# Okrio/tinyrecurrentunet

Measured on AMD Instinct MI355X. Metric: 16 kHz frames/sec (train step), higher is better.
Workload: dtype f32; 1 GPU; config/tiny.json TRU-Net (C_in=4 incl. PCEN), 64 x 4 s 16 kHz pairs per GPU, n_fft 512 hop 128, full fp32 train step; mfma=fp32 forward, bf16x3 backward, fp32_mfma=bf16x3-bwd, frames_per_gpu=32064, global_batch=64, parallelism=dp1

## Files before the change

tinyrecurrentunet_amd/csrc/elementwise.hip:

```cpp
#include <stdlib.h>
#include "common.hpp"

namespace {

__global__ void to_frames_last_kernel(const float* __restrict__ x, float* __restrict__ y, int N, int R, int NP) {
    __shared__ float t[32][33];
    const int n0 = blockIdx.x * 32, r0 = blockIdx.y * 32;
    const int tx = threadIdx.x, ty = threadIdx.y;
    for (int i = ty; i < 32; i += 8) {
        int n = n0 + i, r = r0 + tx;
        t[i][tx] = (n < N && r < R) ? x[(size_t)n * R + r] : 0.f;
    }
    __syncthreads();
    for (int i = ty; i < 32; i += 8) {
        int r = r0 + i, n = n0 + tx;
        if (r < R && n < NP) y[(size_t)r * NP + n] = t[tx][i];
    }
}

__global__ void from_frames_last_kernel(const float* __restrict__ y, float* __restrict__ x, int N, int R, int NP) {
    __shared__ float t[32][33];
    const int n0 = blockIdx.x * 32, r0 = blockIdx.y * 32;
    const int tx = threadIdx.x, ty = threadIdx.y;
    for (int i = ty; i < 32; i += 8) {
        int r = r0 + i, n = n0 + tx;
        t[i][tx] = (r < R && n < NP) ? y[(size_t)r * NP + n] : 0.f;
    }
    __syncthreads();
    for (int i = ty; i < 32; i += 8) {
        int n = n0 + i, r = r0 + tx;
        if (n < N && r < R) x[(size_t)n * R + r] = t[tx][i];
    }
}

__global__ void from_frames_last_affine_kernel(const float* __restrict__ y, float* __restrict__ x, int N, int R, int NP,
                                               int L, const float* __restrict__ scale, const float* __restrict__ shift,
                                               float lo) {
    __shared__ float t[32][33];
    const int n0 = blockIdx.x * 32, r0 = blockIdx.y * 32;
    const int tx = threadIdx.x, ty = threadIdx.y;
    for (int i = ty; i < 32; i += 8) {
        int r = r0 + i, n = n0 + tx;
        float v = 0.f;
        if (r < R && n < NP) {
            const int c = r / L;
            v = fmaxf(fmaf(y[(size_t)r * NP + n], scale[c], shift[c]), lo);
        }
        t[i][tx] = v;
    }
    __syncthreads();
    for (int i = ty; i < 32; i += 8) {
        int n = n0 + i, r = r0 + tx;
        if (n < N && r < R) x[(size_t)n * R + r] = t[tx][i];
    }
}

template <int CIN, int K>
__global__ __launch_bounds__(256) void conv_first_kernel(const float* __restrict__ x, const float* __restrict__ w,
                                                         const float* __restrict__ b, float* __restrict__ y, int Cout,
                                                         int S, int Lin, int Lout, int NP) {
    const int f4 = threadIdx.x;
    const int lo = blockIdx.y * 8 + threadIdx.y;
    const size_t n = (size_t)blockIdx.x * 128 + 4 * f4;
    if (lo >= Lout) return;
    f32x4 xv[CIN][K];
#pragma unroll
    for (int ci = 0; ci < CIN; ++ci)
#pragma unroll
        for (int k = 0; k < K; ++k) {
            int li = lo * S + k - S / 2;
            f32x4 z = {0.f, 0.f, 0.f, 0.f};
            xv[ci][k] = (li >= 0 && li < Lin) ? *(const f32x4*)(x + ((size_t)ci * Lin + li) * NP + n) : z;
        }
    for (int co = 0; co < Cout; ++co) {
        const float bb = b[co];
        f32x4 acc = {bb, bb, bb, bb};
#pragma unroll
        for (int ci = 0; ci < CIN; ++ci)
#pragma unroll
            for (int k = 0; k < K; ++k) {
                const float wv = w[(co * CIN + ci) * K + k];
#pragma unroll
                for (int e = 0; e < 4; ++e) acc[e] = fmaf(wv, xv[ci][k][e], acc[e]);
            }
#pragma unroll
        for (int e = 0; e < 4; ++e) acc[e] = fmaxf(acc[e], 0.f);
#ifdef TRUNET_THIN_NT
        __builtin_nontemporal_store(acc, (f32x4*)(y + ((size_t)co * Lout + lo) * NP + n));
#else
        *(f32x4*)(y + ((size_t)co * Lout + lo) * NP + n) = acc;
#endif
    }
}

constexpr int DW_PARTS = 16;

template <int K>
__global__ __launch_bounds__(256) void dwconv_fwd_kernel(const float* __restrict__ zin, const float* __restrict__ s_in,
                                                         const float* __restrict__ t_in, const float* __restrict__ w,
                                                         const float* __restrict__ b, float* __restrict__ zout,
                                                         float* __restrict__ partials, int C, int S, int Lin, int Lout,
                                                         int NP, int N) {
    __shared__ double red[256];
    const int c = blockIdx.y;
    const int f4 = threadIdx.x & 31, ly = threadIdx.x >> 5;
    const float sc = s_in[c], sh = t_in[c], bb = b[c];
    float wk[K];
#pragma unroll
    for (int k = 0; k < K; ++k) wk[k] = w[c * K + k];
    const int ntn = NP / 128;
    const int items = Lout * ntn;
    float s1 = 0.f, s2 = 0.f;
    for (int it = blockIdx.x * 8 + ly; it < items; it += gridDim.x * 8) {
        const int nt = it / Lout, lo = it - nt * Lout;
// ... 17 lines not shown
    double r2 = block_sum_f64((double)s2, red);
    if (threadIdx.x == 0) {
        partials[((size_t)blockIdx.x * C + c) * 2 + 0] = (float)r1;
        partials[((size_t)blockIdx.x * C + c) * 2 + 1] = (float)r2;
    }
}

template <int K>
__global__ __launch_bounds__(256) void dwconv_bwd_kernel(
    const float* __restrict__ dy, const float* __restrict__ z, const float* __restrict__ ca,
    const float* __restrict__ cb, const float* __restrict__ cc, const float* __restrict__ zin,
    const float* __restrict__ s_in, const float* __restrict__ t_in, const float* __restrict__ mean_in,
    const float* __restrict__ w, float* __restrict__ dy_in, float* __restrict__ partials_in,
    float* __restrict__ w_partials, float* __restrict__ b_partials, int C, int S, int Lin, int Lout, int NP, int N) {
    __shared__ double red[256];
    const int c = blockIdx.y;
    const int f4 = threadIdx.x & 31, ly = threadIdx.x >> 5;
    const float a0 = ca[c], a1 = cb[c], a2 = cc[c];
    const float sc = s_in[c], sh = t_in[c], mu = mean_in[c];
    float wk[K], dwk[K];
#pragma unroll
    for (int k = 0; k < K; ++k) { wk[k] = w[c * K + k]; dwk[k] = 0.f; }
    float db = 0.f, s1 = 0.f, s2 = 0.f;
    const int ntn = NP / 128;
    const int items = Lin * ntn;
    for (int it = blockIdx.x * 8 + ly; it < items; it += gridDim.x * 8) {
        const int nt = it / Lin, li = it - nt * Lin;
        const int n = nt * 128 + 4 * f4;
        const f32x4 zi = *(const f32x4*)(zin + ((size_t)c * Lin + li) * NP + n);
        f32x4 act, g = {0.f, 0.f, 0.f, 0.f};
#pragma unroll
        for (int e = 0; e < 4; ++e) act[e] = fmaxf(fmaf(zi[e], sc, sh), 0.f);
#pragma unroll
        for (int k = 0; k < K; ++k) {
            const int num = li + K / 2 - k;
            const int lo = num / S;
            if (num >= 0 && lo * S == num && lo < Lout) {
                const size_t off = ((size_t)c * Lout + lo) * NP + n;
                const f32x4 dv = *(const f32x4*)(dy + off);
                const f32x4 zv = *(const f32x4*)(z + off);
#pragma unroll
                for (int e = 0; e < 4; ++e) {
                    float dz = (n + e < N) ? fmaf(a0, dv[e], fmaf(a1, zv[e], a2)) : 0.f;
                    g[e] = fmaf(wk[k], dz, g[e]);
                    dwk[k] = fmaf(dz, act[e], dwk[k]);
                    if (k == K / 2) db += dz;
                }
            }
        }
        f32x4 o;
#pragma unroll
        for (int e = 0; e < 4; ++e) {
            o[e] = (act[e] > 0.f) ? g[e] : 0.f;
            s1 += o[e];
            s2 = fmaf(o[e], zi[e] - mu, s2);
        }
        *(f32x4*)(dy_in + ((size_t)c * Lin + li) * NP + n) = o;
    }
    double r;
    r = block_sum_f64((double)s1, red);
    if (threadIdx.x == 0) partials_in[((size_t)blockIdx.x * C + c) * 2 + 0] = (float)r;
    r = block_sum_f64((double)s2, red);
    if (threadIdx.x == 0) partials_in[((size_t)blockIdx.x * C + c) * 2 + 1] = (float)r;
    r = block_sum_f64((double)db, red);
    if (threadIdx.x == 0) b_partials[(size_t)blockIdx.x * C + c] = (float)r;
#pragma unroll
    for (int k = 0; k < K; ++k) {
        r = block_sum_f64((double)dwk[k], red);
        if (threadIdx.x == 0) w_partials[((size_t)blockIdx.x * C + c) * K + k] = (float)r;
    }
}

constexpr int DW2_FB = 32;
constexpr int DW2_CH = 4;
constexpr int DW2_PARTS = DW2_FB * DW2_CH;

#ifndef TRUNET_DW_TEMPORAL
#define DW2_LD(p) __builtin_nontemporal_load((const f32x4*)(p))
#define DW2_ST(p, v) __builtin_nontemporal_store((v), (f32x4*)(p))
#else
#define DW2_LD(p) (*(const f32x4*)(p))
#define DW2_ST(p, v) (*(f32x4*)(p) = (v))
#endif
template <int K, int S>
__global__ __launch_bounds__(256) void dw2_fwd_kernel(const float* __restrict__ zin, const float* __restrict__ s_in,
                                                      const float* __restrict__ t_in, const float* __restrict__ w,
                                                      const float* __restrict__ b, float* __restrict__ zout,
                                                      float* __restrict__ partials, int C, int Lin, int Lout, int NP, int N) {
    __shared__ double red[256];
    const int c = blockIdx.y;
    const float sc = s_in[c], sh = t_in[c], bb = b[c];
    float wk[K];
#pragma unroll
    for (int k = 0; k < K; ++k) wk[k] = w[c * K + k];
    const int lo0 = (int)(((long long)blockIdx.z * Lout) / DW2_CH), lo1 = (int)(((long long)(blockIdx.z + 1) * Lout) / DW2_CH);
    double s1 = 0.0, s2 = 0.0;
    for (int qd = blockIdx.x * 256 + threadIdx.x; qd < NP / 4; qd += DW2_FB * 256) {
        const int n = 4 * qd;
        const float* src = zin + (size_t)c * Lin * NP + n;
        float* dst = zout + (size_t)c * Lout * NP + n;
        auto load_act = [&](int li) {
            f32x4 a = {0.f, 0.f, 0.f, 0.f};
            if (li >= 0 && li < Lin) {
                const f32x4 v = DW2_LD(src + (size_t)li * NP);
#pragma unroll
                for (int e = 0; e < 4; ++e) a[e] = fmaxf(fmaf(v[e], sc, sh), 0.f);
            }
            return a;
        };
        f32x4 win[K];
#pragma unroll
        for (int k = 0; k < K - S; ++k) win[k + S] = load_act(lo0 * S + k - K / 2);
        for (int lo = lo0; lo < lo1; ++lo) {
#pragma unroll
            for (int k = 0; k < K - S; ++k) win[k] = win[k + S];
#pragma unroll
            for (int k = K - S; k < K; ++k) win[k] = load_act(lo * S + k - K / 2);
            f32x4 acc = {bb, bb, bb, bb};
#pragma unroll
            for (int k = 0; k < K; ++k)
#pragma unroll
                for (int e = 0; e < 4; ++e) acc[e] = fmaf(wk[k], win[k][e], acc[e]);
            DW2_ST(dst + (size_t)lo * NP, acc);
            float r1 = 0.f, r2 = 0.f;
#pragma unroll
            for (int e = 0; e < 4; ++e)
                if (n + e < N) { r1 += acc[e]; r2 = fmaf(acc[e], acc[e], r2); }
            s1 += (double)r1;
            s2 += (double)r2;
        }
    }
    const int part = blockIdx.z * DW2_FB + blockIdx.x;
    const double r1 = block_sum_f64(s1, red);
    const double r2 = block_sum_f64(s2, red);
    if (threadIdx.x == 0) {
        partials[((size_t)part * C + c) * 2 + 0] = (float)r1;
        partials[((size_t)part * C + c) * 2 + 1] = (float)r2;
    }
}

template <int K, int S>
__global__ __launch_bounds__(256) void dw2_bwd_kernel(
    const float* __restrict__ dy, const float* __restrict__ z, const float* __restrict__ ca,
    const float* __restrict__ cb, const float* __restrict__ cc, const float* __restrict__ zin,
    const float* __restrict__ s_in, const float* __restrict__ t_in, const float* __restrict__ mean_in,
    const float* __restrict__ w, float* __restrict__ dy_in, float* __restrict__ partials_in,
    float* __restrict__ w_partials, float* __restrict__ b_partials, int C, int Lin, int Lout, int NP, int N) {
    constexpr int LOMIN = -1, LOMAX = 1, W = 3;
    static_assert((K == 3 && S == 1) || (K == 5 && S == 2) || (K == 3 && S == 2), "window derived for these shapes");
    __shared__ double red[256];
    const int c = blockIdx.y;
    const float a0 = ca[c], a1 = cb[c], a2 = cc[c];
    const float sc = s_in[c], sh = t_in[c], mu = mean_in[c];
    float wk[K];
    double dwk[K];
#pragma unroll
    for (int k = 0; k < K; ++k) { wk[k] = w[c * K + k]; dwk[k] = 0.0; }
    double db = 0.0, s1 = 0.0, s2 = 0.0;
    const int G = (Lin + S - 1) / S;
    const int m0 = (int)(((long long)blockIdx.z * G) / DW2_CH), m1 = (int)(((long long)(blockIdx.z + 1) * G) / DW2_CH);
    for (int qd = blockIdx.x * 256 + threadIdx.x; qd < NP / 4; qd += DW2_FB * 256) {
        const int n = 4 * qd;
        const float* pdy = dy + (size_t)c * Lout * NP + n;
        const float* pz = z + (size_t)c * Lout * NP + n;
        const float* pin = zin + (size_t)c * Lin * NP + n;
        float* pout = dy_in + (size_t)c * Lin * NP + n;
        auto load_dz = [&](int lo) {
            f32x4 d = {0.f, 0.f, 0.f, 0.f};
            if (lo >= 0 && lo < Lout) {
                const f32x4 dv = DW2_LD(pdy + (size_t)lo * NP);
                const f32x4 zv = DW2_LD(pz + (size_t)lo * NP);
#pragma unroll
                for (int e = 0; e < 4; ++e) d[e] = (n + e < N) ? fmaf(a0, dv[e], fmaf(a1, zv[e], a2)) : 0.f;
            }
            return d;
        };
        f32x4 dzw[W];
#pragma unroll
        for (int i = 1; i < W; ++i) dzw[i] = load_dz(m0 + LOMIN + i - 1);
        for (int m = m0; m < m1; ++m) {
#pragma unroll
            for (int i = 0; i < W - 1; ++i) dzw[i] = dzw[i + 1];
            dzw[W - 1] = load_dz(m + LOMAX);
#pragma unroll
            for (int e = 0; e < S; ++e) {
                const int li = m * S + e;
                if (li >= Lin) continue;
                const f32x4 zi = DW2_LD(pin + (size_t)li * NP);
                f32x4 act, g = {0.f, 0.f, 0.f, 0.f};
#pragma unroll
                for (int j = 0; j < 4; ++j) act[j] = fmaxf(fmaf(zi[j], sc, sh), 0.f);
#pragma unroll
                for (int k = 0; k < K; ++k) {
                    constexpr int half = K / 2;
                    const int num = e + half - k;
                    if (((num % S) + S) % S != 0) continue;
                    const int lo_rel = (num >= 0) ? num / S : -((-num) / S);
                    const int wi = lo_rel - LOMIN;
                    float rw = 0.f, rb = 0.f;
#pragma unroll
                    for (int j = 0; j < 4; ++j) {
                        const float dzv = dzw[wi][j];
                        g[j] = fmaf(wk[k], dzv, g[j]);
                        rw = fmaf(dzv, act[j], rw);
                        rb += dzv;
                    }
                    dwk[k] += (double)rw;
                    if (k == half) db += (double)rb;
                }
                f32x4 o;
                float r1 = 0.f, r2 = 0.f;
#pragma unroll
                for (int j = 0; j < 4; ++j) {
                    o[j] = (act[j] > 0.f) ? g[j] : 0.f;
                    r1 += o[j];
                    r2 = fmaf(o[j], zi[j] - mu, r2);
                }
                s1 += (double)r1;
                s2 += (double)r2;
                DW2_ST(pout + (size_t)li * NP, o);
            }
        }
    }
    const int part = blockIdx.z * DW2_FB + blockIdx.x;
    double r;
    r = block_sum_f64(s1, red);
    if (threadIdx.x == 0) partials_in[((size_t)part * C + c) * 2 + 0] = (float)r;
    r = block_sum_f64(s2, red);
    if (threadIdx.x == 0) partials_in[((size_t)part * C + c) * 2 + 1] = (float)r;
    r = block_sum_f64(db, red);
    if (threadIdx.x == 0) b_partials[(size_t)part * C + c] = (float)r;
#pragma unroll
    for (int k = 0; k < K; ++k) {
        r = block_sum_f64(dwk[k], red);
        if (threadIdx.x == 0) w_partials[((size_t)part * C + c) * K + k] = (float)r;
    }
}

template <int K, int S>
__global__ __launch_bounds__(256) void dw2_bwd_rz_kernel(
    const float* __restrict__ dy, const float* __restrict__ bias, const float* __restrict__ ca,
    const float* __restrict__ cb, const float* __restrict__ cc, const float* __restrict__ zin,
    const float* __restrict__ s_in, const float* __restrict__ t_in, const float* __restrict__ mean_in,
    const float* __restrict__ w, float* __restrict__ dy_in, float* __restrict__ partials_in,
    float* __restrict__ w_partials, float* __restrict__ b_partials, int C, int Lin, int Lout, int NP, int N) {
    constexpr int LOMIN = -1, W = 3;
    constexpr int AW = S + K / 2 + 1, ZO = S - K / 2;
    static_assert((K == 3 && S == 1) || (K == 5 && S == 2) || (K == 3 && S == 2), "window derived for these shapes");
    __shared__ double red[256];
    const int c = blockIdx.y;
    const float a0 = ca[c], a1 = cb[c], a2 = cc[c];
    const float sc = s_in[c], sh = t_in[c], mu = mean_in[c], bb = bias[c];
    const bool sc0 = fabsf(sc) < 1e-30f || fabsf(sh) > 65536.f * fabsf(sc);
    const float isc = sc0 ? 0.f : 1.f / sc, zoff = fmaf(sh, isc, mu);
    float wk[K];
    double dwk[K];
#pragma unroll
    for (int k = 0; k < K; ++k) { wk[k] = w[c * K + k]; dwk[k] = 0.0; }
    double db = 0.0, s1 = 0.0, s2 = 0.0;
    const int G = (Lin + S - 1) / S;
    const int m0 = (int)(((long long)blockIdx.z * G) / DW2_CH), m1 = (int)(((long long)(blockIdx.z + 1) * G) / DW2_CH);
    for (int qd = blockIdx.x * 256 + threadIdx.x; qd < NP / 4; qd += DW2_FB * 256) {
        const int n = 4 * qd;
        const float* pdy = dy + (size_t)c * Lout * NP + n;
        const float* pin = zin + (size_t)c * Lin * NP + n;
        float* pout = dy_in + (size_t)c * Lin * NP + n;
        f32x4 aw[AW];
        auto load_row = [&](int li, f32x4& act) {
            const bool ok = li >= 0 && li < Lin;
            const f32x4 raw = DW2_LD(pin + (size_t)min(max(li, 0), Lin - 1) * NP);
#pragma unroll
            for (int j = 0; j < 4; ++j) act[j] = ok ? fmaxf(fmaf(raw[j], sc, sh), 0.f) : 0.f;
        };
        f32x4 dzw[W];
#pragma unroll
        for (int i = 0; i < W; ++i) dzw[i] = f32x4{0.f, 0.f, 0.f, 0.f};
        const int ms = m0 - 2;
#pragma unroll
        for (int i = S; i < AW; ++i) load_row(ms * S + i - S, aw[i]);
        for (int m = ms; m < m1; ++m) {
#pragma unroll
            for (int i = 0; i < AW - S; ++i) aw[i] = aw[i + S];
#pragma unroll
            for (int i = AW - S; i < AW; ++i) load_row(m * S + i, aw[i]);
#pragma unroll
            for (int i = 0; i < W - 1; ++i) dzw[i] = dzw[i + 1];
            {
                const int lo = m + 1;
                const bool ok = lo >= 0 && lo < Lout;
                const f32x4 dv = DW2_LD(pdy + (size_t)min(max(lo, 0), Lout - 1) * NP);
                f32x4 zrec = {bb, bb, bb, bb};
#pragma unroll
                for (int k = 0; k < K; ++k)
#pragma unroll
                    for (int j = 0; j < 4; ++j) zrec[j] = fmaf(wk[k], aw[ZO + k][j], zrec[j]);
#pragma unroll
                for (int j = 0; j < 4; ++j)
                    dzw[W - 1][j] = (ok && n + j < N) ? fmaf(a0, dv[j], fmaf(a1, zrec[j], a2)) : 0.f;
            }
            if (m < m0) continue;
#pragma unroll
            for (int e = 0; e < S; ++e) {
                const int li = m * S + e;
                if (li >= Lin) continue;
                const f32x4 act = aw[e];
                f32x4 zc;
#pragma unroll
                for (int j = 0; j < 4; ++j) zc[j] = fmaf(act[j], isc, -zoff);
                if (sc0) {
                    const f32x4 zi = DW2_LD(pin + (size_t)li * NP);
#pragma unroll
                    for (int j = 0; j < 4; ++j) zc[j] = zi[j] - mu;
                }
                f32x4 g = {0.f, 0.f, 0.f, 0.f};
#pragma unroll
                for (int k = 0; k < K; ++k) {
                    constexpr int half = K / 2;
                    const int num = e + half - k;
                    if (((num % S) + S) % S != 0) continue;
                    const int lo_rel = (num >= 0) ? num / S : -((-num) / S);
                    const int wi = lo_rel - LOMIN;
                    float rw = 0.f, rb = 0.f;
#pragma unroll
                    for (int j = 0; j < 4; ++j) {
                        const float dzv = dzw[wi][j];
                        g[j] = fmaf(wk[k], dzv, g[j]);
                        rw = fmaf(dzv, act[j], rw);
                        rb += dzv;
                    }
                    dwk[k] += (double)rw;
                    if (k == half) db += (double)rb;
                }
                f32x4 o;
                float r1 = 0.f, r2 = 0.f;
#pragma unroll
                for (int j = 0; j < 4; ++j) {
                    o[j] = (act[j] > 0.f) ? g[j] : 0.f;
                    r1 += o[j];
                    r2 = fmaf(o[j], zc[j], r2);
                }
                s1 += (double)r1;
                s2 += (double)r2;
                DW2_ST(pout + (size_t)li * NP, o);
            }
        }
    }
    const int part = blockIdx.z * DW2_FB + blockIdx.x;
    double r;
    r = block_sum_f64(s1, red);
    if (threadIdx.x == 0) partials_in[((size_t)part * C + c) * 2 + 0] = (float)r;
    r = block_sum_f64(s2, red);
    if (threadIdx.x == 0) partials_in[((size_t)part * C + c) * 2 + 1] = (float)r;
    r = block_sum_f64(db, red);
    if (threadIdx.x == 0) b_partials[(size_t)part * C + c] = (float)r;
#pragma unroll
    for (int k = 0; k < K; ++k) {
        r = block_sum_f64(dwk[k], red);
        if (threadIdx.x == 0) w_partials[((size_t)part * C + c) * K + k] = (float)r;
    }
}

__global__ __launch_bounds__(256) void relu_bwd_stats_kernel(float* __restrict__ dy, const float* __restrict__ z,
                                                             const float* __restrict__ sc, const float* __restrict__ sh,
                                                             const float* __restrict__ mean, float* __restrict__ partials,
                                                             int C, int L, int NP, int N) {
    __shared__ double red[256];
    const int c = blockIdx.y;
    const int f4 = threadIdx.x & 31, ly = threadIdx.x >> 5;
    const float a0 = sc ? sc[c] : 1.f, a1 = sc ? sh[c] : 0.f, mu = mean ? mean[c] : 0.f;
    const int ntn = NP / 128;
    const int items = L * ntn;
    float s1 = 0.f, s2 = 0.f;
    for (int it = blockIdx.x * 8 + ly; it < items; it += gridDim.x * 8) {
        const int nt = it / L, l = it - nt * L;
        const int n = nt * 128 + 4 * f4;
        const size_t off = ((size_t)c * L + l) * NP + n;
        f32x4 d = *(const f32x4*)(dy + off);
        const f32x4 zv = *(const f32x4*)(z + off);
#pragma unroll
        for (int e = 0; e < 4; ++e) {
            d[e] = (n + e < N && fmaf(zv[e], a0, a1) > 0.f) ? d[e] : 0.f;
            s1 += d[e];
            s2 = fmaf(d[e], (n + e < N) ? zv[e] - mu : 0.f, s2);
        }
        *(f32x4*)(dy + off) = d;
    }
    if (partials) {
        double r = block_sum_f64((double)s1, red);
        if (threadIdx.x == 0) partials[((size_t)blockIdx.x * C + c) * 2 + 0] = (float)r;
        r = block_sum_f64((double)s2, red);
        if (threadIdx.x == 0) partials[((size_t)blockIdx.x * C + c) * 2 + 1] = (float)r;
    }
}

__global__ __launch_bounds__(256) void gru_cell_kernel(const float* __restrict__ gi, const float* __restrict__ gh,
                                                       const float* h, float* hn, int H,
                                                      
                                                       size_t R4) {
    const size_t i = (size_t)blockIdx.x * 256 + threadIdx.x;
    if (i >= (size_t)H * R4) return;
    const size_t HR = (size_t)H * R4;
    const f32x4* gi4 = (const f32x4*)gi;
    const f32x4* gh4 = (const f32x4*)gh;
    const f32x4 ir = gi4[i], iz = gi4[HR + i], in_ = gi4[2 * HR + i];
    const f32x4 hr = gh4[i], hz = gh4[HR + i], hn_ = gh4[2 * HR + i];
    const f32x4 hp = ((const f32x4*)h)[i];
    f32x4 o;
#pragma unroll
    for (int e = 0; e < 4; ++e) {
        const float r = 1.f / (1.f + expf(-(ir[e] + hr[e])));
        const float z = 1.f / (1.f + expf(-(iz[e] + hz[e])));
        const float n = tanhf(in_[e] + r * hn_[e]);
        o[e] = (1.f - z) * n + z * hp[e];
    }
    ((f32x4*)hn)[i] = o;
}

__global__ void to_seq_major_kernel(const float* __restrict__ x, float* __restrict__ y, const float* __restrict__ sc,
                                    const float* __restrict__ sh, int Lf, int T, int B, int NP, int SP, float lo) {
    __shared__ float tl[32][33];
    const int c = blockIdx.z / Lf, l = blockIdx.z % Lf;
    const int t0 = blockIdx.x * 32, b0 = blockIdx.y * 32;
    const int tx = threadIdx.x, ty = threadIdx.y;
    const float a0 = sc ? sc[c] : 1.f, a1 = sc ? sh[c] : 0.f;
    for (int i = ty; i < 32; i += 8) {
        const int b = b0 + i, t = t0 + tx;
        float v = 0.f;
        if (b < B && t < T) v = fmaxf(fmaf(x[((size_t)c * Lf + l) * NP + (size_t)b * T + t], a0, a1), lo);
// ... 184 lines not shown
    for (int g = threadIdx.x; g < nparts; g += 256) {
        f32x2* pp = (f32x2*)(partials + ((size_t)g * C + c) * 2);
        const f32x2 v = *pp;
        a += (double)v[0];
        b += (double)v[1];
        *pp = f32x2{0.f, 0.f};
    }
    a = block_sum_f64(a, red);
    b = block_sum_f64(b, red);
    if (threadIdx.x == 0) {
        const double r = rstd[c], g = gamma[c], mu = mean[c];
        const double m1 = a / count;
        const double m2 = r * b / count;
        dgamma[c] = (float)(r * b);
        dbeta[c] = (float)a;
        ca[c] = (float)(g * r);
        cb[c] = (float)(-g * r * r * m2);
        cc[c] = (float)(-g * r * m1 + g * r * r * m2 * mu);
    }
}

__global__ void adamw_kernel(float* __restrict__ p, const float* __restrict__ g, float* __restrict__ m,
                             float* __restrict__ v, int64_t n, float lr, float b1, float b2, float eps, float wd,
                             float bc1, float bc2_sqrt) {
    int64_t i = (int64_t)blockIdx.x * blockDim.x + threadIdx.x;
    if (i >= n) return;
    float gi = g[i];
    float pi = p[i] * (1.f - lr * wd);
    float mi = b1 * m[i] + (1.f - b1) * gi;
    float vi = b2 * v[i] + (1.f - b2) * gi * gi;
    m[i] = mi;
    v[i] = vi;
    float denom = sqrtf(vi) / bc2_sqrt + eps;
    p[i] = pi - (lr / bc1) * (mi / denom);
}

__global__ __launch_bounds__(1024) void sumsq_kernel(const float* __restrict__ g, int64_t n, float* out) {
    __shared__ double red[1024];
    const int tid = threadIdx.x;
    double s0 = 0.0, s1 = 0.0, s2 = 0.0, s3 = 0.0;
    const int64_t n4 = ((reinterpret_cast<uintptr_t>(g) & 15) == 0) ? n / 4 : 0;
    const f32x4* g4 = (const f32x4*)g;
    for (int64_t i = tid; i < n4; i += 1024) {
        const f32x4 v = g4[i];
        s0 += (double)v[0] * (double)v[0];
        s1 += (double)v[1] * (double)v[1];
        s2 += (double)v[2] * (double)v[2];
        s3 += (double)v[3] * (double)v[3];
    }
    for (int64_t i = 4 * n4 + tid; i < n; i += 1024) s0 += (double)g[i] * (double)g[i];
    red[tid] = (s0 + s1) + (s2 + s3);
    __syncthreads();
    for (int w = 512; w > 0; w >>= 1) {
        if (tid < w) red[tid] += red[tid + w];
        __syncthreads();
    }
    if (tid == 0) out[0] = (float)red[0];
}

struct ChecksumDesc { const uint32_t* ptr; long long nwords; };
__global__ __launch_bounds__(256) void checksum_batch_kernel(const ChecksumDesc* __restrict__ desc, unsigned long long* out) {
    __shared__ unsigned long long red[256];
    const ChecksumDesc d = desc[blockIdx.y];
    unsigned long long acc = 0ull;
    for (long long i = (long long)blockIdx.x * 256 + threadIdx.x; i < d.nwords; i += (long long)gridDim.x * 256) {
        unsigned long long h = (unsigned long long)d.ptr[i] + 0x9E3779B97F4A7C15ull * (unsigned long long)(i + 1) +
                               0xC2B2AE3D27D4EB4Full * (unsigned long long)(blockIdx.y + 1);
        h ^= h >> 31; h *= 0x7FB5D329728EA185ull; h ^= h >> 27; h *= 0x81DADEF4BC2DD44Dull; h ^= h >> 33;
        acc += h;
    }
    red[threadIdx.x] = acc;
    __syncthreads();
    for (int s = 128; s > 0; s >>= 1) {
        if (threadIdx.x < s) red[threadIdx.x] += red[threadIdx.x + s];
        __syncthreads();
    }
    if (threadIdx.x == 0 && red[0]) atomicAdd(out, red[0]);
}

}

#define ST ((hipStream_t)stream)

extern "C" int trunet_to_frames_last(const float* x, float* y, int N, int C, int L, int NP, void* stream) {
    if (!x || !y || N <= 0 || NP < N) return TRUNET_EINVAL;
    int R = C * L;
    hipLaunchKernelGGL(to_frames_last_kernel, dim3((NP + 31) / 32, (R + 31) / 32), dim3(32, 8), 0, ST, x, y, N, R, NP);
    return trunet_launch_status();
}

extern "C" int trunet_from_frames_last(const float* x, float* y, int N, int C, int L, int NP, void* stream) {
    if (!x || !y || N <= 0 || NP < N) return TRUNET_EINVAL;
    int R = C * L;
    hipLaunchKernelGGL(from_frames_last_kernel, dim3((NP + 31) / 32, (R + 31) / 32), dim3(32, 8), 0, ST, x, y, N, R, NP);
    return trunet_launch_status();
}

extern "C" int trunet_gru_cell(const float* gi, const float* gh, const float* h, float* h_new, int H, int L, int NP,
                               void* stream) {
    if (!gi || !gh || !h || !h_new || H <= 0 || L <= 0 || NP <= 0 || (NP % 4)) return TRUNET_EINVAL;
    const size_t R4 = (size_t)L * NP / 4;
    const size_t n = (size_t)H * R4;
    hipLaunchKernelGGL(gru_cell_kernel, dim3((unsigned)((n + 255) / 256)), dim3(256), 0, ST, gi, gh, h, h_new, H, R4);
    return trunet_launch_status();
}

extern "C" int trunet_to_seq_major(const float* x, float* y, const float* scale, const float* shift, int relu, int C,
                                   int Lf, int T, int B, int NP, int SP, void* stream) {
    if (!x || !y || C <= 0 || Lf <= 0 || T <= 0 || B <= 0 || (size_t)B * T > (size_t)NP || B * Lf > SP) return TRUNET_EINVAL;
    if (hipMemsetAsync(y, 0, (size_t)C * T * SP * sizeof(float), ST) != hipSuccess) return TRUNET_ELAUNCH;
    hipLaunchKernelGGL(to_seq_major_kernel, dim3((T + 31) / 32, (B + 31) / 32, C * Lf), dim3(32, 8), 0, ST, x, y, scale,
                       shift, Lf, T, B, NP, SP, (scale && relu) ? 0.f : -3.0e38f);
    return trunet_launch_status();
}

extern "C" int trunet_from_seq_major_nparts(int Lf, int T, int B) { return ((T + 31) / 32) * ((B + 31) / 32) * Lf; }

extern "C" int trunet_from_seq_major(const float* y, float* x, const float* zsrc, const float* scale, const float* shift,
                                     const float* mean, float* partials, int C, int Lf, int T, int B, int NP, int SP,
                                     void* stream) {
    if (!x || !y || C <= 0 || Lf <= 0 || T <= 0 || B <= 0 || (size_t)B * T > (size_t)NP || B * Lf > SP) return TRUNET_EINVAL;
    if (zsrc && (!scale || !shift || !mean || !partials)) return TRUNET_EINVAL;
    hipLaunchKernelGGL(from_seq_major_kernel, dim3((T + 31) / 32, (B + 31) / 32, C * Lf), dim3(32, 8), 0, ST, y, x, zsrc,
                       scale, shift, mean, partials, C, Lf, T, B, NP, SP);
    return trunet_launch_status();
}

extern "C" int trunet_tgru_cell_fwd(const float* gi_all, const float* gh, float* hs, float* gates, int H, int T, int t,
                                    int SP, void* stream) {
    if (!gi_all || !gh || !hs || H <= 0 || T <= 0 || t < 0 || t >= T || SP <= 0 || (SP % 4)) return TRUNET_EINVAL;
    const size_t n = (size_t)H * (SP / 4);
    hipLaunchKernelGGL(tgru_cell_fwd_kernel, dim3((unsigned)((n + 255) / 256)), dim3(256), 0, ST, gi_all, gh, hs, gates, H,
                       T, t, SP);
    return trunet_launch_status();
}

extern "C" int trunet_tgru_cell_bwd(float* dhs, const float* carry, const float* hs, const float* gates, float* dgi_all,
                                    float* dgh_all, int H, int T, int t, int SP, int S, void* stream) {
    if (!dhs || !hs || !gates || !dgi_all || !dgh_all || H <= 0 || T <= 0 || t < 0 || t >= T || SP <= 0 || (SP % 4))
        return TRUNET_EINVAL;
    const size_t n = (size_t)H * (SP / 4);
    hipLaunchKernelGGL(tgru_cell_bwd_kernel, dim3((unsigned)((n + 255) / 256)), dim3(256), 0, ST, dhs, carry, hs, gates,
                       dgi_all, dgh_all, H, T, t, SP, S);
    return trunet_launch_status();
}

extern "C" int trunet_from_frames_last_affine(const float* x, float* y, int N, int C, int L, int NP, const float* scale,
                                              const float* shift, int relu, void* stream) {
    if (!x || !y || !scale || !shift || N <= 0 || NP < N) return TRUNET_EINVAL;
    int R = C * L;
    hipLaunchKernelGGL(from_frames_last_affine_kernel, dim3((NP + 31) / 32, (R + 31) / 32), dim3(32, 8), 0, ST, x, y, N, R,
                       NP, L, scale, shift, relu ? 0.f : -3.0e38f);
    return trunet_launch_status();
}

extern "C" int trunet_conv_first_fwd(const float* x, const float* w, const float* b, float* y, int Cin, int Cout, int K,
                                     int S, int Lin, int Lout, int NP, void* stream) {
    if (!x || !w || !b || !y || (NP % 128)) return TRUNET_EINVAL;
    dim3 grid(NP / 128, (Lout + 7) / 8), block(32, 8);
    if (K == 5 && Cin == 3) hipLaunchKernelGGL((conv_first_kernel<3, 5>), grid, block, 0, ST, x, w, b, y, Cout, S, Lin, Lout, NP);
    else if (K == 5 && Cin == 4) hipLaunchKernelGGL((conv_first_kernel<4, 5>), grid, block, 0, ST, x, w, b, y, Cout, S, Lin, Lout, NP);
    else return TRUNET_ENOTSUP;
    return trunet_launch_status();
}

static bool dw_gather_forced() {
    static const bool v = [] { const char* e = getenv("TRUNET_DW_GATHER"); return e && e[0] == '1'; }();
    return v;
}

extern "C" int trunet_dwconv_nparts(int Lout) { (void)Lout; return DW2_PARTS; }
extern "C" int trunet_dwconv_bwd_nparts(int Lin) { (void)Lin; return DW2_PARTS; }

extern "C" int trunet_dwconv_fwd(const float* zin, const float* s_in, const float* t_in, const float* w, const float* b,
                                 float* zout, float* partials, int C, int K, int S, int Lin, int Lout, int NP, int N,
                                 void* stream) {
    if (!zin || !s_in || !t_in || !w || !b || !zout || !partials || (NP % 128)) return TRUNET_EINVAL;
    if (!dw_gather_forced() && Lout == (Lin + 2 * (K / 2) - K) / S + 1 &&
        ((K == 3 && S == 1) || (K == 5 && S == 2) || (K == 3 && S == 2))) {
        const dim3 g2(DW2_FB, C, DW2_CH);
#define DW2_FWD(KK, SS) hipLaunchKernelGGL((dw2_fwd_kernel<KK, SS>), g2, dim3(256), 0, ST, zin, s_in, t_in, w, b, zout, partials, C, \
                                           Lin, Lout, NP, N)
        if (K == 3 && S == 1) DW2_FWD(3, 1);
        else if (K == 5) DW2_FWD(5, 2);
        else DW2_FWD(3, 2);
#undef DW2_FWD
        return trunet_launch_status();
    }
    dim3 grid(DW2_PARTS, C);
    if (K == 3) hipLaunchKernelGGL(dwconv_fwd_kernel<3>, grid, dim3(256), 0, ST, zin, s_in, t_in, w, b, zout, partials, C, S, Lin, Lout, NP, N);
    else if (K == 5) hipLaunchKernelGGL(dwconv_fwd_kernel<5>, grid, dim3(256), 0, ST, zin, s_in, t_in, w, b, zout, partials, C, S, Lin, Lout, NP, N);
    else return TRUNET_ENOTSUP;
    return trunet_launch_status();
}

extern "C" int trunet_dwconv_bwd(const float* dy, const float* z, const float* ca, const float* cb, const float* cc,
                                 const float* zin, const float* s_in, const float* t_in, const float* mean_in,
                                 const float* w, float* dy_in, float* partials_in, float* w_partials, float* b_partials,
                                 int C, int K, int S, int Lin, int Lout, int NP, int N, void* stream) {
    if (!dy || !z || !ca || !cb || !cc || !zin || !s_in || !t_in || !mean_in || !w || !dy_in || !partials_in ||
        !w_partials || !b_partials || (NP % 128))
        return TRUNET_EINVAL;
    if (!dw_gather_forced() && Lout == (Lin + 2 * (K / 2) - K) / S + 1 &&
        ((K == 3 && S == 1) || (K == 5 && S == 2) || (K == 3 && S == 2))) {
        const dim3 g2(DW2_FB, C, DW2_CH);
#define DW2_BWD(KK, SS) hipLaunchKernelGGL((dw2_bwd_kernel<KK, SS>), g2, dim3(256), 0, ST, dy, z, ca, cb, cc, zin, s_in, t_in,   \
                                           mean_in, w, dy_in, partials_in, w_partials, b_partials, C, Lin, Lout, NP, N)
        if (K == 3 && S == 1) DW2_BWD(3, 1);
        else if (K == 5) DW2_BWD(5, 2);
        else DW2_BWD(3, 2);
#undef DW2_BWD
        return trunet_launch_status();
    }
    dim3 grid(DW2_PARTS, C);
    if (K == 3) hipLaunchKernelGGL(dwconv_bwd_kernel<3>, grid, dim3(256), 0, ST, dy, z, ca, cb, cc, zin, s_in, t_in, mean_in, w, dy_in, partials_in, w_partials, b_partials, C, S, Lin, Lout, NP, N);
    else if (K == 5) hipLaunchKernelGGL(dwconv_bwd_kernel<5>, grid, dim3(256), 0, ST, dy, z, ca, cb, cc, zin, s_in, t_in, mean_in, w, dy_in, partials_in, w_partials, b_partials, C, S, Lin, Lout, NP, N);
    else return TRUNET_ENOTSUP;
    return trunet_launch_status();
}

extern "C" int trunet_dwconv_bwd_rz(const float* dy, const float* bias, const float* ca, const float* cb, const float* cc,
                                    const float* zin, const float* s_in, const float* t_in, const float* mean_in,
                                    const float* w, float* dy_in, float* partials_in, float* w_partials, float* b_partials,
                                    int C, int K, int S, int Lin, int Lout, int NP, int N, void* stream) {
    if (!dy || !bias || !ca || !cb || !cc || !zin || !s_in || !t_in || !mean_in || !w || !dy_in || !partials_in ||
        !w_partials || !b_partials || (NP % 128))
        return TRUNET_EINVAL;
    static const bool off = [] { const char* e = getenv("TRUNET_DW_RZ"); return e && e[0] == '0'; }();
    if (off || dw_gather_forced() || Lout != (Lin + 2 * (K / 2) - K) / S + 1 ||
        !((K == 3 && S == 1) || (K == 5 && S == 2) || (K == 3 && S == 2)))
        return TRUNET_ENOTSUP;
    if (Lout < 32 && !(getenv("TRUNET_DW_RZ") && getenv("TRUNET_DW_RZ")[0] == '2')) return TRUNET_ENOTSUP;
    const dim3 g2(DW2_FB, C, DW2_CH);
#define DW2_BWD(KK, SS) hipLaunchKernelGGL((dw2_bwd_rz_kernel<KK, SS>), g2, dim3(256), 0, ST, dy, bias, ca, cb, cc, zin, s_in,  \
                                           t_in, mean_in, w, dy_in, partials_in, w_partials, b_partials, C, Lin, Lout, NP, N)
    if (K == 3 && S == 1) DW2_BWD(3, 1);
    else if (K == 5) DW2_BWD(5, 2);
    else DW2_BWD(3, 2);
#undef DW2_BWD
    return trunet_launch_status();
}

extern "C" int trunet_relu_bwd_stats_nparts(void) { return DW_PARTS; }

extern "C" int trunet_relu_bwd_stats(float* dy, const float* z, const float* scale, const float* shift, const float* mean,
                                     float* partials, int C, int L, int NP, int N, void* stream) {
    if (!dy || !z || C <= 0 || L <= 0 || N <= 0 || NP < N || (NP % 128)) return TRUNET_EINVAL;
    if ((scale == nullptr) != (shift == nullptr) || (mean != nullptr) != (partials != nullptr)) return TRUNET_EINVAL;
    hipLaunchKernelGGL(relu_bwd_stats_kernel, dim3(DW_PARTS, C), dim3(256), 0, ST, dy, z, scale, shift, mean, partials, C,
                       L, NP, N);
    return trunet_launch_status();
}

extern "C" int trunet_bn_finalize_fwd(float* partials, int nparts, int C, double count, const float* gamma,
                                      const float* beta, float eps, float momentum, float* running_mean,
                                      float* running_var, float* scale, float* shift, float* mean, float* rstd,
                                      int64_t* num_batches_tracked, void* stream) {
    if (!partials || !gamma || !beta || !scale || !shift || !mean || !rstd || C <= 0 || nparts <= 0) return TRUNET_EINVAL;
    if ((running_mean == nullptr) != (running_var == nullptr)) return TRUNET_EINVAL;
    hipLaunchKernelGGL(bn_finalize_fwd_kernel, dim3(C), dim3(256), 0, ST, partials, nparts, C, count, gamma, beta, eps,
                       momentum, running_mean, running_var, scale, shift, mean, rstd, (long long*)num_batches_tracked);
    return trunet_launch_status();
}

extern "C" int trunet_bn_eval_affine(int C, const float* gamma, const float* beta, const float* running_mean,
                                     const float* running_var, float eps, float* scale, float* shift, void* stream) {
    if (!gamma || !beta || !running_mean || !running_var || !scale || !shift) return TRUNET_EINVAL;
    hipLaunchKernelGGL(bn_eval_affine_kernel, dim3((C + 127) / 128), dim3(128), 0, ST, C, gamma, beta, running_mean,
                       running_var, eps, scale, shift);
    return trunet_launch_status();
}

extern "C" int trunet_bn_finalize_bwd(float* partials, int nparts, int C, double count, const float* gamma,
                                      const float* mean, const float* rstd, float* dgamma, float* dbeta, float* ca,
                                      float* cb, float* cc, void* stream) {
    if (!partials || !gamma || !mean || !rstd || !dgamma || !dbeta || !ca || !cb || !cc) return TRUNET_EINVAL;
    hipLaunchKernelGGL(bn_finalize_bwd_kernel, dim3(C), dim3(256), 0, ST, partials, nparts, C, count, gamma, mean, rstd,
                       dgamma, dbeta, ca, cb, cc);
    return trunet_launch_status();
}

extern "C" int trunet_adamw(float* p, const float* g, float* m, float* v, int64_t n, float lr, float beta1, float beta2,
                            float eps, float wd, int step, void* stream) {
    if (!p || !g || !m || !v || n <= 0 || step < 1) return TRUNET_EINVAL;
    float bc1 = 1.f - powf(beta1, (float)step);
    float bc2s = sqrtf(1.f - powf(beta2, (float)step));
    hipLaunchKernelGGL(adamw_kernel, dim3((unsigned)((n + 255) / 256)), dim3(256), 0, ST, p, g, m, v, n, lr, beta1, beta2,
                       eps, wd, bc1, bc2s);
    return trunet_launch_status();
}

extern "C" int trunet_checksum_batch(const void* desc, int n, uint64_t* out, void* stream) {
    if (!desc || !out || n <= 0 || n > 65535) return TRUNET_EINVAL;
    hipLaunchKernelGGL(checksum_batch_kernel, dim3(8, n), dim3(256), 0, ST, (const ChecksumDesc*)desc, (unsigned long long*)out);
    return trunet_launch_status();
}

extern "C" int trunet_sumsq(const float* g, int64_t n, float* out, void* stream) {
    if (!g || !out || n <= 0) return TRUNET_EINVAL;
    hipLaunchKernelGGL(sumsq_kernel, dim3(1), dim3(1024), 0, ST, g, n, out);
    return trunet_launch_status();
}

namespace {
__global__ __launch_bounds__(256) void mfma_peak_kernel(float* out, int iters, float seed) {
    f32x16 acc[4];
#pragma unroll
    for (int t = 0; t < 4; ++t)
#pragma unroll
        for (int r = 0; r < 16; ++r) acc[t][r] = 0.f;
    float a = seed + threadIdx.x * 1e-3f, b = seed * 0.5f + threadIdx.x * 2e-3f;
    for (int i = 0; i < iters; ++i) {
#pragma unroll
        for (int u = 0; u < 4; ++u) {
#pragma unroll
            for (int t = 0; t < 4; ++t) acc[t] = __builtin_amdgcn_mfma_f32_32x32x2f32(a, b, acc[t], 0, 0, 0);
        }
// ... 16 lines not shown
```

Before: 778,000 frames/s.

## Software-pipeline depthwise conv row loads and vectorize frames-last transposes

Adds a generic register-level software pipeline that issues the global loads for the next row(s) before computing the current one. It is used in the depthwise conv forward, backward and recompute-backward kernels, with per-shape depths chosen at compile time. Separately, the frames-last transpose kernels get 64x64 tiled versions with 16-byte vector loads and stores when alignment allows. The aim is to hide memory latency in bandwidth-bound elementwise stages, at the cost of more registers and some redundant clamped loads at the tails.

After: 774,800 frames/s. No clear change (-0.4%).

```diff
diff --git a/tinyrecurrentunet_amd/csrc/elementwise.hip b/tinyrecurrentunet_amd/csrc/elementwise.hip
--- a/tinyrecurrentunet_amd/csrc/elementwise.hip
+++ b/tinyrecurrentunet_amd/csrc/elementwise.hip
@@ -30,6 +30,56 @@
     for (int i = ty; i < 32; i += 8) {
         int n = n0 + i, r = r0 + tx;
         if (n < N && r < R) x[(size_t)n * R + r] = t[tx][i];
+    }
+}
+
+constexpr int FL4_T = 64, FL4_LD = FL4_T + 1;
+
+__global__ __launch_bounds__(256) void to_frames_last_v4_kernel(const float* __restrict__ x, float* __restrict__ y, int N,
+                                                                int R, int NP) {
+    __shared__ float t[FL4_T][FL4_LD];
+    const int n0 = blockIdx.x * FL4_T, r0 = blockIdx.y * FL4_T;
+    const int q = threadIdx.x & 15, h = threadIdx.x >> 4;
+#pragma unroll
+    for (int i = 0; i < 4; ++i) {
+        const int n = n0 + h + 16 * i, r = r0 + 4 * q;
+        f32x4 v = {0.f, 0.f, 0.f, 0.f};
+        if (n < N && r < R) v = *(const f32x4*)(x + (size_t)n * R + r);
+#pragma unroll
+        for (int e = 0; e < 4; ++e) t[h + 16 * i][4 * q + e] = v[e];
+    }
+    __syncthreads();
+#pragma unroll
+    for (int i = 0; i < 4; ++i) {
+        const int r = r0 + h + 16 * i, n = n0 + 4 * q;
+        f32x4 v;
+#pragma unroll
+        for (int e = 0; e < 4; ++e) v[e] = t[4 * q + e][h + 16 * i];
+        if (r < R && n < NP) *(f32x4*)(y + (size_t)r * NP + n) = v;
+    }
+}
+
+__global__ __launch_bounds__(256) void from_frames_last_v4_kernel(const float* __restrict__ y, float* __restrict__ x, int N,
+                                                                  int R, int NP) {
+    __shared__ float t[FL4_T][FL4_LD];
+    const int n0 = blockIdx.x * FL4_T, r0 = blockIdx.y * FL4_T;
+    const int q = threadIdx.x & 15, h = threadIdx.x >> 4;
+#pragma unroll
+    for (int i = 0; i < 4; ++i) {
+        const int r = r0 + h + 16 * i, n = n0 + 4 * q;
+        f32x4 v = {0.f, 0.f, 0.f, 0.f};
+        if (r < R && n < NP) v = *(const f32x4*)(y + (size_t)r * NP + n);
+#pragma unroll
+        for (int e = 0; e < 4; ++e) t[h + 16 * i][4 * q + e] = v[e];
+    }
+    __syncthreads();
+#pragma unroll
+    for (int i = 0; i < 4; ++i) {
+        const int n = n0 + h + 16 * i, r = r0 + 4 * q;
+        f32x4 v;
+#pragma unroll
+        for (int e = 0; e < 4; ++e) v[e] = t[4 * q + e][h + 16 * i];
+        if (n < N && r < R) *(f32x4*)(x + (size_t)n * R + r) = v;
     }
 }
 
@@ -213,7 +263,40 @@
 #define DW2_LD(p) (*(const f32x4*)(p))
 #define DW2_ST(p, v) (*(f32x4*)(p) = (v))
 #endif
-template <int K, int S>
+#ifndef TRUNET_DW_NOPIPE
+#ifndef TRUNET_DW_DEPTHS
+#define TRUNET_DW_DEPTHS 1, 1, 1, 1, 0, 1
+#endif
+#else
+#undef TRUNET_DW_DEPTHS
+#define TRUNET_DW_DEPTHS 0, 0, 0, 0, 0, 0
+#endif
+constexpr int DW2_DEPTHS[6] = {TRUNET_DW_DEPTHS};
+constexpr int dw2_fwd_depth(int K, int S) { return DW2_DEPTHS[K == 5 ? 1 : S == 2 ? 2 : 0]; }
+constexpr int dw2_bwd_rz_depth(int K, int S) { return K == 5 ? DW2_DEPTHS[4] : S == 1 ? DW2_DEPTHS[3] : 0; }
+constexpr int dw2_bwd_depth(int K, int S) { return (K == 3 && S == 2) ? DW2_DEPTHS[5] : 0; }
+template <int V> struct dw2_ic { static constexpr int value = V; };
+
+template <int D, int W, class Req, class Step>
+__device__ __forceinline__ void dw2_pipeline(int i0, int i1, Req request, Step step) {
+    constexpr int U = D + 1;
+    f32x4 set[U][W];
+#pragma unroll
+    for (int d = 0; d < D; ++d) request(i0 + d, set[d]);
+    int i = i0;
+    for (; i + U <= i1; i += U) {
+#pragma unroll
+        for (int u = 0; u < U; ++u) {
+            request(i + u + D, set[(u + D) % U]);
+            step(i + u, set[u]);
+        }
+    }
+#pragma unroll
+    for (int u = 0; u < D; ++u)
+        if (i + u < i1) step(i + u, set[u]);
+}
+
+template <int K, int S, int D>
 __global__ __launch_bounds__(256) void dw2_fwd_kernel(const float* __restrict__ zin, const float* __restrict__ s_in,
                                                       const float* __restrict__ t_in, const float* __restrict__ w,
                                                       const float* __restrict__ b, float* __restrict__ zout,
@@ -242,11 +325,7 @@
         f32x4 win[K];
 #pragma unroll
         for (int k = 0; k < K - S; ++k) win[k + S] = load_act(lo0 * S + k - K / 2);
-        for (int lo = lo0; lo < lo1; ++lo) {
-#pragma unroll
-            for (int k = 0; k < K - S; ++k) win[k] = win[k + S];
-#pragma unroll
-            for (int k = K - S; k < K; ++k) win[k] = load_act(lo * S + k - K / 2);
+        auto finish = [&](int lo) {
             f32x4 acc = {bb, bb, bb, bb};
 #pragma unroll
             for (int k = 0; k < K; ++k)
@@ -259,6 +338,35 @@
                 if (n + e < N) { r1 += acc[e]; r2 = fmaf(acc[e], acc[e], r2); }
             s1 += (double)r1;
             s2 += (double)r2;
+        };
+        if constexpr (D > 0) {
+            const int li_last = min((lo1 - 1) * S + K - 1 - K / 2, Lin - 1);
+            auto request = [&](int lo, f32x4* raw) {
+#pragma unroll
+                for (int k = 0; k < S; ++k)
+                    raw[k] = DW2_LD(src + (size_t)max(min(lo * S + K - S + k - K / 2, li_last), 0) * NP);
+            };
+            auto step = [&](int lo, const f32x4* raw) {
+#pragma unroll
+                for (int k = 0; k < K - S; ++k) win[k] = win[k + S];
+#pragma unroll
+                for (int k = 0; k < S; ++k) {
+                    const int li = lo * S + K - S + k - K / 2;
+                    const bool ok = li >= 0 && li < Lin;
+#pragma unroll
+                    for (int e = 0; e < 4; ++e) win[K - S + k][e] = ok ? fmaxf(fmaf(raw[k][e], sc, sh), 0.f) : 0.f;
+                }
+                finish(lo);
+            };
+            dw2_pipeline<D, S>(lo0, lo1, request, step);
+        } else {
+            for (int lo = lo0; lo < lo1; ++lo) {
+#pragma unroll
+                for (int k = 0; k < K - S; ++k) win[k] = win[k + S];
+#pragma unroll
+                for (int k = K - S; k < K; ++k) win[k] = load_act(lo * S + k - K / 2);
+                finish(lo);
+            }
         }
     }
     const int part = blockIdx.z * DW2_FB + blockIdx.x;
@@ -270,7 +378,7 @@
     }
 }
 
-template <int K, int S>
+template <int K, int S, int D>
 __global__ __launch_bounds__(256) void dw2_bwd_kernel(
     const float* __restrict__ dy, const float* __restrict__ z, const float* __restrict__ ca,
     const float* __restrict__ cb, const float* __restrict__ cc, const float* __restrict__ zin,
@@ -296,60 +404,86 @@
         const float* pz = z + (size_t)c * Lout * NP + n;
         const float* pin = zin + (size_t)c * Lin * NP + n;
         float* pout = dy_in + (size_t)c * Lin * NP + n;
+        auto dz_row = [&](const f32x4& dv, const f32x4& zv) {
+            f32x4 d;
+#pragma unroll
+            for (int e = 0; e < 4; ++e) d[e] = (n + e < N) ? fmaf(a0, dv[e], fmaf(a1, zv[e], a2)) : 0.f;
+            return d;
+        };
         auto load_dz = [&](int lo) {
             f32x4 d = {0.f, 0.f, 0.f, 0.f};
-            if (lo >= 0 && lo < Lout) {
-                const f32x4 dv = DW2_LD(pdy + (size_t)lo * NP);
-                const f32x4 zv = DW2_LD(pz + (size_t)lo * NP);
-#pragma unroll
-                for (int e = 0; e < 4; ++e) d[e] = (n + e < N) ? fmaf(a0, dv[e], fmaf(a1, zv[e], a2)) : 0.f;
-            }
+            if (lo >= 0 && lo < Lout) d = dz_row(DW2_LD(pdy + (size_t)lo * NP), DW2_LD(pz + (size_t)lo * NP));
             return d;
         };
         f32x4 dzw[W];
+        auto in_row = [&](auto ec, int li, const f32x4& zi) {
+            constexpr int e = decltype(ec)::value;
+            f32x4 act, g = {0.f, 0.f, 0.f, 0.f};
+#pragma unroll
+            for (int j = 0; j < 4; ++j) act[j] = fmaxf(fmaf(zi[j], sc, sh), 0.f);
+#pragma unroll
+            for (int k = 0; k < K; ++k) {
+                constexpr int half = K / 2;
+                const int num = e + half - k;
+                if (((num % S) + S) % S != 0) continue;
+                const int lo_rel = (num >= 0) ? num / S : -((-num) / S);
+                const int wi = lo_rel - LOMIN;
+                float rw = 0.f, rb = 0.f;
+#pragma unroll
+                for (int j = 0; j < 4; ++j) {
+                    const float dzv = dzw[wi][j];
+                    g[j] = fmaf(wk[k], dzv, g[j]);
+                    rw = fmaf(dzv, act[j], rw);
+                    rb += dzv;
+                }
+                dwk[k] += (double)rw;
+                if (k == half) db += (double)rb;
+            }
+            f32x4 o;
+            float r1 = 0.f, r2 = 0.f;
+#pragma unroll
+            for (int j = 0; j < 4; ++j) {
+                o[j] = (act[j] > 0.f) ? g[j] : 0.f;
+                r1 += o[j];
+                r2 = fmaf(o[j], zi[j] - mu, r2);
+            }
+            s1 += (double)r1;
+            s2 += (double)r2;
+            DW2_ST(pout + (size_t)li * NP, o);
+        };
 #pragma unroll
         for (int i = 1; i < W; ++i) dzw[i] = load_dz(m0 + LOMIN + i - 1);
-        for (int m = m0; m < m1; ++m) {
-#pragma unroll
-            for (int i = 0; i < W - 1; ++i) dzw[i] = dzw[i + 1];
-            dzw[W - 1] = load_dz(m + LOMAX);
-#pragma unroll
-            for (int e = 0; e < S; ++e) {
-                const int li = m * S + e;
-                if (li >= Lin) continue;
-                const f32x4 zi = DW2_LD(pin + (size_t)li * NP);
-                f32x4 act, g = {0.f, 0.f, 0.f, 0.f};
-#pragma unroll
-                for (int j = 0; j < 4; ++j) act[j] = fmaxf(fmaf(zi[j], sc, sh), 0.f);
-#pragma unroll
-                for (int k = 0; k < K; ++k) {
-                    constexpr int half = K / 2;
-                    const int num = e + half - k;
-                    if (((num % S) + S) % S != 0) continue;
-                    const int lo_rel = (num >= 0) ? num / S : -((-num) / S);
-                    const int wi = lo_rel - LOMIN;
-                    float rw = 0.f, rb = 0.f;
-#pragma unroll
-                    for (int j = 0; j < 4; ++j) {
-                        const float dzv = dzw[wi][j];
-                        g[j] = fmaf(wk[k], dzv, g[j]);
-                        rw = fmaf(dzv, act[j], rw);
-                        rb += dzv;
-                    }
-                    dwk[k] += (double)rw;
-                    if (k == half) db += (double)rb;
+        if constexpr (D > 0) {
+            auto request = [&](int mm, f32x4* q) {
+                const int m = max(min(mm, m1 - 1), 0);
+                const size_t lo = (size_t)min(m + LOMAX, Lout - 1);
+                q[0] = DW2_LD(pdy + lo * NP);
+                q[1] = DW2_LD(pz + lo * NP);
+#pragma unroll
+                for (int e = 0; e < S; ++e) q[2 + e] = DW2_LD(pin + (size_t)min(m * S + e, Lin - 1) * NP);
+            };
+            auto step = [&](int m, const f32x4* cur) {
+#pragma unroll
+                for (int i = 0; i < W - 1; ++i) dzw[i] = dzw[i + 1];
+                {
+                    const f32x4 d = dz_row(cur[0], cur[1]);
+                    const bool ok = m + LOMAX < Lout;
+#pragma unroll
+                    for (int e = 0; e < 4; ++e) dzw[W - 1][e] = ok ? d[e] : 0.f;
                 }
-                f32x4 o;
-                float r1 = 0.f, r2 = 0.f;
-#pragma unroll
-                for (int j = 0; j < 4; ++j) {
-                    o[j] = (act[j] > 0.f) ? g[j] : 0.f;
-                    r1 += o[j];
-                    r2 = fmaf(o[j], zi[j] - mu, r2);
-                }
-                s1 += (double)r1;
-                s2 += (double)r2;
-                DW2_ST(pout + (size_t)li * NP, o);
+                in_row(dw2_ic<0>{}, m * S, cur[2]);
+                if constexpr (S == 2)
+                    if (m * S + 1 < Lin) in_row(dw2_ic<1>{}, m * S + 1, cur[3]);
+            };
+            dw2_pipeline<D, S + 2>(m0, m1, request, step);
+        } else {
+            for (int m = m0; m < m1; ++m) {
+#pragma unroll
+                for (int i = 0; i < W - 1; ++i) dzw[i] = dzw[i + 1];
+                dzw[W - 1] = load_dz(m + LOMAX);
+                in_row(dw2_ic<0>{}, m * S, DW2_LD(pin + (size_t)(m * S) * NP));
+                if constexpr (S == 2)
+                    if (m * S + 1 < Lin) in_row(dw2_ic<1>{}, m * S + 1, DW2_LD(pin + (size_t)(m * S + 1) * NP));
             }
         }
     }
@@ -368,7 +502,7 @@
     }
 }
 
-template <int K, int S>
+template <int K, int S, int D>
 __global__ __launch_bounds__(256) void dw2_bwd_rz_kernel(
     const float* __restrict__ dy, const float* __restrict__ bias, const float* __restrict__ ca,
     const float* __restrict__ cb, const float* __restrict__ cc, const float* __restrict__ zin,
@@ -397,29 +531,36 @@
         const float* pin = zin + (size_t)c * Lin * NP + n;
         float* pout = dy_in + (size_t)c * Lin * NP + n;
         f32x4 aw[AW];
-        auto load_row = [&](int li, f32x4& act) {
+        auto load_raw = [&](int li) { return DW2_LD(pin + (size_t)min(max(li, 0), Lin - 1) * NP); };
+        auto activate = [&](int li, const f32x4& raw, f32x4& act) {
             const bool ok = li >= 0 && li < Lin;
-            const f32x4 raw = DW2_LD(pin + (size_t)min(max(li, 0), Lin - 1) * NP);
 #pragma unroll
             for (int j = 0; j < 4; ++j) act[j] = ok ? fmaxf(fmaf(raw[j], sc, sh), 0.f) : 0.f;
         };
+        auto load_row = [&](int li, f32x4& act) { activate(li, load_raw(li), act); };
+        auto request = [&](int mm, f32x4* q) {
+            const int m = min(mm, m1 - 1);
+#pragma unroll
+            for (int i = 0; i < S; ++i) q[i] = load_raw(m * S + AW - S + i);
+            q[S] = DW2_LD(pdy + (size_t)min(max(m + 1, 0), Lout - 1) * NP);
+        };
         f32x4 dzw[W];
 #pragma unroll
         for (int i = 0; i < W; ++i) dzw[i] = f32x4{0.f, 0.f, 0.f, 0.f};
         const int ms = m0 - 2;
 #pragma unroll
         for (int i = S; i < AW; ++i) load_row(ms * S + i - S, aw[i]);
-        for (int m = ms; m < m1; ++m) {
+        auto step = [&](int m, const f32x4* cur) {
 #pragma unroll
             for (int i = 0; i < AW - S; ++i) aw[i] = aw[i + S];
 #pragma unroll
-            for (int i = AW - S; i < AW; ++i) load_row(m * S + i, aw[i]);
+            for (int i = AW - S; i < AW; ++i) activate(m * S + i, cur[i - (AW - S)], aw[i]);
 #pragma unroll
             for (int i = 0; i < W - 1; ++i) dzw[i] = dzw[i + 1];
             {
                 const int lo = m + 1;
                 const bool ok = lo >= 0 && lo < Lout;
-                const f32x4 dv = DW2_LD(pdy + (size_t)min(max(lo, 0), Lout - 1) * NP);
+                const f32x4 dv = cur[S];
                 f32x4 zrec = {bb, bb, bb, bb};
 #pragma unroll
                 for (int k = 0; k < K; ++k)
@@ -429,7 +570,7 @@
                 for (int j = 0; j < 4; ++j)
                     dzw[W - 1][j] = (ok && n + j < N) ? fmaf(a0, dv[j], fmaf(a1, zrec[j], a2)) : 0.f;
             }
-            if (m < m0) continue;
+            if (m < m0) return;
 #pragma unroll
             for (int e = 0; e < S; ++e) {
                 const int li = m * S + e;
@@ -474,7 +615,8 @@
                 s2 += (double)r2;
                 DW2_ST(pout + (size_t)li * NP, o);
             }
-        }
+        };
+        dw2_pipeline<D, S + 1>(ms, m1, request, step);
     }
     const int part = blockIdx.z * DW2_FB + blockIdx.x;
     double r;
@@ -825,17 +967,33 @@
 
 #define ST ((hipStream_t)stream)
 
+static bool frames_last_v4(const void* a, const void* b, int R, int NP) {
+#ifdef TRUNET_DW_NOPIPE
+    return false;
+#else
+    return R % 4 == 0 && NP % 4 == 0 && (((uintptr_t)a | (uintptr_t)b) & 15) == 0;
+#endif
+}
+
 extern "C" int trunet_to_frames_last(const float* x, float* y, int N, int C, int L, int NP, void* stream) {
     if (!x || !y || N <= 0 || NP < N) return TRUNET_EINVAL;
     int R = C * L;
-    hipLaunchKernelGGL(to_frames_last_kernel, dim3((NP + 31) / 32, (R + 31) / 32), dim3(32, 8), 0, ST, x, y, N, R, NP);
+    if (frames_last_v4(x, y, R, NP))
+        hipLaunchKernelGGL(to_frames_last_v4_kernel, dim3((NP + FL4_T - 1) / FL4_T, (R + FL4_T - 1) / FL4_T), dim3(256), 0, ST,
+                           x, y, N, R, NP);
+    else
+        hipLaunchKernelGGL(to_frames_last_kernel, dim3((NP + 31) / 32, (R + 31) / 32), dim3(32, 8), 0, ST, x, y, N, R, NP);
     return trunet_launch_status();
 }
 
 extern "C" int trunet_from_frames_last(const float* x, float* y, int N, int C, int L, int NP, void* stream) {
     if (!x || !y || N <= 0 || NP < N) return TRUNET_EINVAL;
     int R = C * L;
-    hipLaunchKernelGGL(from_frames_last_kernel, dim3((NP + 31) / 32, (R + 31) / 32), dim3(32, 8), 0, ST, x, y, N, R, NP);
+    if (frames_last_v4(x, y, R, NP))
+        hipLaunchKernelGGL(from_frames_last_v4_kernel, dim3((NP + FL4_T - 1) / FL4_T, (R + FL4_T - 1) / FL4_T), dim3(256), 0,
+                           ST, x, y, N, R, NP);
+    else
+        hipLaunchKernelGGL(from_frames_last_kernel, dim3((NP + 31) / 32, (R + 31) / 32), dim3(32, 8), 0, ST, x, y, N, R, NP);
     return trunet_launch_status();
 }
 
@@ -922,7 +1080,7 @@
     if (!dw_gather_forced() && Lout == (Lin + 2 * (K / 2) - K) / S + 1 &&
         ((K == 3 && S == 1) || (K == 5 && S == 2) || (K == 3 && S == 2))) {
         const dim3 g2(DW2_FB, C, DW2_CH);
-#define DW2_FWD(KK, SS) hipLaunchKernelGGL((dw2_fwd_kernel<KK, SS>), g2, dim3(256), 0, ST, zin, s_in, t_in, w, b, zout, partials, C, \
+#define DW2_FWD(KK, SS) hipLaunchKernelGGL((dw2_fwd_kernel<KK, SS, dw2_fwd_depth(KK, SS)>), g2, dim3(256), 0, ST, zin, s_in, t_in, w, b, zout, partials, C, \
                                            Lin, Lout, NP, N)
         if (K == 3 && S == 1) DW2_FWD(3, 1);
         else if (K == 5) DW2_FWD(5, 2);
@@ -947,7 +1105,7 @@
     if (!dw_gather_forced() && Lout == (Lin + 2 * (K / 2) - K) / S + 1 &&
         ((K == 3 && S == 1) || (K == 5 && S == 2) || (K == 3 && S == 2))) {
         const dim3 g2(DW2_FB, C, DW2_CH);
-#define DW2_BWD(KK, SS) hipLaunchKernelGGL((dw2_bwd_kernel<KK, SS>), g2, dim3(256), 0, ST, dy, z, ca, cb, cc, zin, s_in, t_in,   \
+#define DW2_BWD(KK, SS) hipLaunchKernelGGL((dw2_bwd_kernel<KK, SS, dw2_bwd_depth(KK, SS)>), g2, dim3(256), 0, ST, dy, z, ca, cb, cc, zin, s_in, t_in,   \
                                            mean_in, w, dy_in, partials_in, w_partials, b_partials, C, Lin, Lout, NP, N)
         if (K == 3 && S == 1) DW2_BWD(3, 1);
         else if (K == 5) DW2_BWD(5, 2);
@@ -975,7 +1133,7 @@
         return TRUNET_ENOTSUP;
     if (Lout < 32 && !(getenv("TRUNET_DW_RZ") && getenv("TRUNET_DW_RZ")[0] == '2')) return TRUNET_ENOTSUP;
     const dim3 g2(DW2_FB, C, DW2_CH);
-#define DW2_BWD(KK, SS) hipLaunchKernelGGL((dw2_bwd_rz_kernel<KK, SS>), g2, dim3(256), 0, ST, dy, bias, ca, cb, cc, zin, s_in,  \
+#define DW2_BWD(KK, SS) hipLaunchKernelGGL((dw2_bwd_rz_kernel<KK, SS, dw2_bwd_rz_depth(KK, SS)>), g2, dim3(256), 0, ST, dy, bias, ca, cb, cc, zin, s_in,  \
                                            t_in, mean_in, w, dy_in, partials_in, w_partials, b_partials, C, Lin, Lout, NP, N)
     if (K == 3 && S == 1) DW2_BWD(3, 1);
     else if (K == 5) DW2_BWD(5, 2);
```
